# thetisproject/thetis

Hardware: AMD Instinct MI355X
Metric: DG element-updates/sec, 2D SWE DG-P1 SSPRK33 (higher is better)
Workload: dtype f64

## Files before the change

### thetis_amd/csrc/swe2d_api_fuse.hip

```cpp
#include "swe2d_handle.h"
#include "swe2d_fuse.h"

namespace swe2d_impl {

namespace {
typedef void (*fuse_kernel_t)(const SweFuseArgs);
template <bool SRC>
fuse_kernel_t pick_fuse_src(bool nl, bool lf)
{
    if (nl) return lf ? swe_fuse12_kernel<true, true, SRC> : swe_fuse12_kernel<true, false, SRC>;
    return lf ? swe_fuse12_kernel<false, true, SRC> : swe_fuse12_kernel<false, false, SRC>;
}
fuse_kernel_t pick_fuse_kernel(bool nl, bool lf, bool src) { return src ? pick_fuse_src<true>(nl, lf) : pick_fuse_src<false>(nl, lf); }
}

int fuseq_build(Handle *h);
int fuse12_build(Handle *h)
{
    if (h->npc == 4) return fuseq_build(h);
    if (h->fuse_tile || h->fuse_state == -1 || stream_capturing(h)) return SWE2D_OK;
    const int n = h->n_cells;
    const size_t S = h->stride;
    const int *nbr = h->h_nbr.data();
    std::vector<int2> tl;
// ... 128 lines not shown
        const int ni = (int)cells.size();
        for (int c : ring) if (state[c] == 2) cells.push_back(c);
        const int nt = (int)cells.size();
        if (nt - ni != n_ring || nt > SWE_FUSE_WG) return fail(h, SWE2D_ERR_UNSUPPORTED, "fused stage pair: tile bookkeeping");
        for (int l = 0; l < nt; l++) lane_of[cells[l]] = l;
        const size_t base = tl.size();
        tl.resize(base + SWE_FUSE_WG, int4{-1, 0, 0, 0});
        int n_out = 0;
        for (int l = 0; l < nt; l++) {
            const int c = cells[l];
            unsigned w[4];
            for (int f = 0; f < 4; f++) {
                const int code = nbr[(size_t)f*S + c];
                if (code < 0) w[f] = (unsigned)l;
                else if (state[code >> 2] != 0) w[f] = (unsigned)lane_of[code >> 2];
                else {
                    if (l < ni || n_out >= SWE_QFUSE_MAX_OUT) return fail(h, SWE2D_ERR_UNSUPPORTED, "fused stage pair: ring bookkeeping");
                    w[f] = 0x200u | (unsigned)n_out++;
                }
            }
            tl[base + l] = int4{c, (int)(w[0] | (w[1] << SWE_FUSE_FBITS) | (w[2] << (2*SWE_FUSE_FBITS))), (int)w[3], 0};
        }
        inner.push_back(ni);
        n_ring_total += nt - ni;
        for (int c : cells) { state[c] = 0; lane_of[c] = -1; }
    }
    h->fuseq_n_tiles = (int)inner.size();
    if (!fuse12_tiles_pay(h, h->fuseq_n_tiles)) { h->fuse_state = -1; h->fuseq_n_tiles = 0; return SWE2D_OK; }
    HIP_TRY(h, hipMalloc(&h->fuseq_tile, tl.size()*sizeof(int4)));
    HIP_TRY(h, hipMalloc(&h->fuseq_inner, inner.size()*sizeof(int)));
    HIP_TRY(h, hipMemcpy(h->fuseq_tile, tl.data(), tl.size()*sizeof(int4), hipMemcpyHostToDevice));
    HIP_TRY(h, hipMemcpy(h->fuseq_inner, inner.data(), inner.size()*sizeof(int), hipMemcpyHostToDevice));
    h->fuseq_ring_cells = n_ring_total;
    return SWE2D_OK;
}

namespace {
typedef void (*fuseq_kernel_t)(const SweFuseQuadArgs);
template <bool SRC, bool AFFINE>
fuseq_kernel_t pick_fuseq_2(bool nl, bool lf)
{
    if (nl) return lf ? swe_fuse12_quad_kernel<true, true, SRC, AFFINE> : swe_fuse12_quad_kernel<true, false, SRC, AFFINE>;
    return lf ? swe_fuse12_quad_kernel<false, true, SRC, AFFINE> : swe_fuse12_quad_kernel<false, false, SRC, AFFINE>;
}
fuseq_kernel_t pick_fuseq_kernel(bool nl, bool lf, bool src, bool affine)
{
    if (affine) return src ? pick_fuseq_2<true, true>(nl, lf) : pick_fuseq_2<false, true>(nl, lf);
    return src ? pick_fuseq_2<true, false>(nl, lf) : pick_fuseq_2<false, false>(nl, lf);
}
}

int launch_fuse12_quad(Handle *h, int cell_end)
{
    if (!h->fuseq_tile) return fail(h, SWE2D_ERR_UNSUPPORTED, "fused stage pair: no tile tables");
    SweFuseQuadArgs q;
    fill_stage_args(h, q.st, 0, 0, 2, 0.0, 1.0, kBeta[0], 0, h->n_owned);
    q.tile = h->fuseq_tile;
    q.n_inner = h->fuseq_inner;
    q.n_tiles = h->fuseq_n_tiles;
    q.cell_end = cell_end;
    q.beta1 = kBeta[0];
    q.a0_2 = kAlpha0[1]; q.a1_2 = kAlphaIn[1]; q.beta2 = kBeta[1];
    q.out = h->state[2];
    fuseq_kernel_t kern = pick_fuseq_kernel(h->par.use_nonlinear_equations != 0, h->par.use_lax_friedrichs_velocity != 0, has_sources(h), h->affine);
    const int grid = ((h->fuseq_n_tiles + 7)/8)*8;
    SWE_CHK_SYNC(h->stream);
    hipLaunchKernelGGL(kern, dim3(grid), dim3(SWE_FUSE_WG), 0, h->stream, q);
    HIP_TRY(h, hipGetLastError());
    stage_written(h, false, true);
    return SWE2D_OK;
}

namespace {
typedef void (*fuse3_kernel_t)(const SweFuse3Args);
template <bool SRC>
fuse3_kernel_t pick_fuse3_src(bool nl, bool lf)
{
    if (nl) return lf ? swe_fuse123_kernel<true, true, SRC> : swe_fuse123_kernel<true, false, SRC>;
    return lf ? swe_fuse123_kernel<false, true, SRC> : swe_fuse123_kernel<false, false, SRC>;
}
fuse3_kernel_t pick_fuse3_kernel(bool nl, bool lf, bool src) { return src ? pick_fuse3_src<true>(nl, lf) : pick_fuse3_src<false>(nl, lf); }
}

int fuse123_build(Handle *h)
{
    if (h->fuse3_tile || stream_capturing(h)) return SWE2D_OK;
    const int n = h->n_cells;
    const size_t S = h->stride;
    const int *nbr = h->h_nbr.data();
    const int *order = (int)h->fuse3_order.size() == n ? h->fuse3_order.data() : ((int)h->fuse_order.size() == n ? h->fuse_order.data() : nullptr);
    const unsigned char *start = (int)h->fuse3_start.size() == n ? h->fuse3_start.data() : nullptr;
    std::vector<int2> tl, cnt;
    std::vector<unsigned char> state((size_t)n, 0);
    std::vector<int> lane_of((size_t)n, -1), touched, inner;
    std::vector<std::pair<int, unsigned char>> undo;
    int count[4] = {0, 0, 0, 0};
    long long r1_total = 0, r2_total = 0;
    auto set = [&](int c, unsigned char ns) {
        undo.push_back({c, state[c]});
        if (state[c] == 0) touched.push_back(c);
        count[state[c]]--; state[c] = ns; count[ns]++;
    };
    for (int pos = 0; pos < n;) {
        inner.clear(); touched.clear();
        count[1] = count[2] = count[3] = 0;
        while (pos < n) {
            if (start && start[pos] && !inner.empty()) break;
            const int kk = order ? order[pos] : pos;
            undo.clear();
            const size_t touched_before = touched.size();
            set(kk, 1);
            for (int f = 0; f < 3; f++) {
                const int code = nbr[(size_t)f*S + kk];
                if (code < 0) continue;
                const int c1 = code >> 2;
                if (state[c1] == 0 || state[c1] == 3) {
                    set(c1, 2);
                    for (int g = 0; g < 3; g++) {
                        const int code2 = nbr[(size_t)g*S + c1];
                        if (code2 >= 0 && state[code2 >> 2] == 0) set(code2 >> 2, 3);
                    }
                }
            }
            if (count[1] + count[2] + count[3] > SWE_FUSE_WG || 2*count[3] > SWE_FUSE3_MAX_OUT) {
                if (inner.empty()) return fail(h, SWE2D_ERR_UNSUPPORTED, "fused stages: a cell whose two rings do not fit a tile");
                for (size_t i = undo.size(); i-- > 0;) { count[state[undo[i].first]]--; state[undo[i].first] = undo[i].second; count[undo[i].second]++; }
                touched.resize(touched_before);
                break;
            }
            inner.push_back(kk);
            pos++;
        }
        std::vector<int> cells(inner);
        for (int want = 2; want <= 3; want++)
            for (int c : touched) if (state[c] == want) cells.push_back(c);
        const int ni = (int)inner.size(), nm = ni + count[2], nt = (int)cells.size();
        if (nt != count[1] + count[2] + count[3] || ni != count[1] || nt > SWE_FUSE_WG) return fail(h, SWE2D_ERR_UNSUPPORTED, "fused stages: tile bookkeeping");
        for (int l = 0; l < nt; l++) lane_of[cells[l]] = l;
        const size_t base = tl.size();
        tl.resize(base + SWE_FUSE_WG, int2{-1, 0});
        int n_out = 0;
        for (int l = 0; l < nt; l++) {
            const int c = cells[l];
            unsigned w = 0u;
            for (int f = 0; f < 3; f++) {
                const int code = nbr[(size_t)f*S + c];
                unsigned field;
                if (code < 0) field = (unsigned)l;
                else if (state[code >> 2] != 0) field = (unsigned)lane_of[code >> 2];
                else {
                    if (l < nm || n_out >= SWE_FUSE3_MAX_OUT) return fail(h, SWE2D_ERR_UNSUPPORTED, "fused stages: ring bookkeeping");
                    field = 0x200u | (unsigned)n_out++;
                }
                w |= field << (SWE_FUSE_FBITS*f);
            }
            tl[base + l] = int2{c, (int)w};
        }
        cnt.push_back(int2{ni, nm});
        r1_total += count[2]; r2_total += count[3];
        for (int c : cells) { state[c] = 0; lane_of[c] = -1; }
    }
    h->fuse3_n_tiles = (int)cnt.size();
    HIP_TRY(h, hipMalloc(&h->fuse3_tile, tl.size()*sizeof(int2)));
    HIP_TRY(h, hipMalloc(&h->fuse3_cnt, cnt.size()*sizeof(int2)));
    HIP_TRY(h, hipMemcpy(h->fuse3_tile, tl.data(), tl.size()*sizeof(int2), hipMemcpyHostToDevice));
    HIP_TRY(h, hipMemcpy(h->fuse3_cnt, cnt.data(), cnt.size()*sizeof(int2), hipMemcpyHostToDevice));
    h->fuse3_ring1 = r1_total; h->fuse3_ring2 = r2_total;
    return SWE2D_OK;
}

int launch_fuse123(Handle *h, int cell_end)
{
    if (int rc = capture_parity_check(h)) return rc;
    if (int rc = fuse123_build(h)) return rc;
    if (!h->fuse3_tile) return fail(h, SWE2D_ERR_UNSUPPORTED, "fused stages: no tile tables (not built inside a stream capture)");
    SweFuse3Args q;
    fill_stage_args(h, q.st, 0, 0, 1, 0.0, 1.0, kBeta[0], 0, h->n_owned);
    q.st.idxc = h->opt[SWE2D_OPT_COMPACT_IDX] == 0 ? nullptr : h->idxc;
    q.tile = h->fuse3_tile;
    q.counts = h->fuse3_cnt;
    q.n_tiles = h->fuse3_n_tiles;
    q.cell_end = cell_end;
    for (int s = 0; s < 3; s++) { q.a0[s] = s ? kAlpha0[s] : 0.0; q.a1[s] = s ? kAlphaIn[s] : 1.0; q.beta[s] = kBeta[s]; }
    q.out = h->state[1];
    fuse3_kernel_t kern = pick_fuse3_kernel(h->par.use_nonlinear_equations != 0, h->par.use_lax_friedrichs_velocity != 0, has_sources(h));
    const int grid = ((h->fuse3_n_tiles + 7)/8)*8;
    SWE_CHK_SYNC(h->stream);
    hipLaunchKernelGGL(kern, dim3(grid), dim3(SWE_FUSE_WG), 0, h->stream, q);
    HIP_TRY(h, hipGetLastError());
    swap_state_buffers(h);
    unsigned long long id = 0;
    if (stream_capturing(h, &id)) {
        if (id != h->capture_id) { h->capture_id = id; h->capture_swaps = 0; }
        h->capture_swaps++;
    }
    return SWE2D_OK;
}

int capture_parity_check(Handle *h)
{
    if (h->capture_swaps == 0 && h->capture_odd == 0) return SWE2D_OK;
    unsigned long long id = 0;
    const bool capturing = stream_capturing(h, &id);
    if (h->capture_swaps) {
        if (capturing && id == h->capture_id) return SWE2D_OK;
        if (h->capture_swaps & 1) { swap_state_buffers(h); h->capture_odd++; }
        h->capture_swaps = 0;
    }
    if (capturing || h->capture_odd == 0) return SWE2D_OK;
    const int odd = h->capture_odd;
    h->capture_odd = 0;
    return fail(h, SWE2D_ERR_UNSUPPORTED, std::to_string(odd) + " stream capture(s) recorded an odd number of swe2d_solve_step_cells launches: "
                "such a graph ends on the other state buffer than it began on and cannot be replayed (the state is the one from before the "
                "capture); capture an even number per sequence");
}

}

static int checked_tile_order(Handle *h, const int32_t *cells, std::vector<int> &order)
{
    std::vector<char> seen((size_t)h->n_cells, 0);
    for (int i = 0; cells && i < h->n_cells; i++) {
        if (cells[i] < 0 || cells[i] >= h->n_cells || seen[cells[i]]) return fail(h, SWE2D_ERR_INVALID_ARGUMENT, "fused stages: the tile order is not a permutation of the cells");
        seen[cells[i]] = 1;
    }
    if (cells) order.assign(cells, cells + h->n_cells);
    return SWE2D_OK;
}

extern "C" {

int swe2d_fused_set_order(swe2d_handle *hh, const int32_t *cells_in_tile_order)
{
    Handle *h = H(hh);
    if (!h) return SWE2D_ERR_INVALID_ARGUMENT;
    HIP_TRY(h, hipSetDevice(h->device));
    std::vector<int> order;
    if (int rc = checked_tile_order(h, cells_in_tile_order, order)) return rc;
    HIP_TRY(h, hipStreamSynchronize(h->stream));
    if (h->fuse_tile) { (void)hipFree(h->fuse_tile); h->fuse_tile = nullptr; }
    if (h->fuse_inner) { (void)hipFree(h->fuse_inner); h->fuse_inner = nullptr; }
// ... 80 lines not shown
```

### thetis_amd/csrc/swe2d_flow.h

```cpp
#pragma once
#include "swe2d_kernels.h"
#include "swe2d_p2p.h"

#ifndef SWE_FLOW_OCCUPANCY
#define SWE_FLOW_OCCUPANCY __attribute__((amdgpu_waves_per_eu(2, 2)))
#endif
#define SWE_FLOW_MAX_STAGES 384
#define SWE_FLOW_MAX_CYCLES 64
#ifndef SWE_FLOW_FLAG_STRIDE
#define SWE_FLOW_FLAG_STRIDE 16
#endif
#define SWE_FLOW_SLOT_BYTES 128
#define SWE_FLOW_DIV6(t_) ((int)(((unsigned)(t_)*43691u) >> 18))
#ifndef SWE_FLOW_POLL_SLEEP
#define SWE_FLOW_POLL_SLEEP 2
#endif
#ifndef SWE_FLOW_NTR_SRC
#define SWE_FLOW_NTR_SRC 3
#endif
#ifndef SWE_FLOW_WALLFAST_SRC
#define SWE_FLOW_WALLFAST_SRC true
#endif
#ifndef SWE_FLOW_RX
#define SWE_FLOW_RX 3
// ... 72 lines not shown
    while (wall_clock64() - t0 < (unsigned long long)ticks) __builtin_amdgcn_s_sleep(16);
    if (aux_sys) __builtin_amdgcn_raw_buffer_store_b64(lo2, r, off, 0, 17); else __builtin_amdgcn_raw_buffer_store_b64(lo2, r, off, 0, 16);
}
#define SWE_FLOW_TORN(lb_, pc_, sys_) ((swe_flow_tear[0] == (lb_) || swe_flow_tear[0] == -2) && swe_flow_tear[1] > 0 \
                                       && ((pc_) % (swe_flow_tear[2] < 1 ? 1 : swe_flow_tear[2])) == 0 && (!(sys_) || swe_flow_tear[3]))
#endif
__device__ __forceinline__ void swe_flow_put(__amdgpu_buffer_rsrc_t r, unsigned off, double x, unsigned tag, bool torn = false)
{
    const swe_u32x2 xb = __builtin_bit_cast(swe_u32x2, x);
    const swe_u32x4 g = {xb.x, xb.y, tag, swe_flow_check_word(xb.x, xb.y, tag)};
#ifdef SWE_FLOW_TEAR
    if (torn) { swe_flow_put_torn(r, off, g, 0, swe_flow_tear[1]); return; }
#endif
    (void)torn;
    __builtin_amdgcn_raw_buffer_store_b128(g, r, off, 0, 16);
}
__device__ __forceinline__ swe_u32x4 swe_flow_get(__amdgpu_buffer_rsrc_t r, unsigned off)
{
    return __builtin_amdgcn_raw_buffer_load_b128(r, off, 0, 16);
}
__device__ __forceinline__ void swe_flow_put_sys(__amdgpu_buffer_rsrc_t r, unsigned off, double x, unsigned tag, bool torn = false)
{
    const swe_u32x2 xb = __builtin_bit_cast(swe_u32x2, x);
    const swe_u32x4 g = {xb.x, xb.y, tag, swe_flow_check_word(xb.x, xb.y, tag)};
#ifdef SWE_FLOW_TEAR
    if (torn) { swe_flow_put_torn(r, off, g, 1, swe_flow_tear[1]); return; }
#endif
    (void)torn;
    __builtin_amdgcn_raw_buffer_store_b128(g, r, off, 0, 17);
}
__device__ __forceinline__ swe_u32x4 swe_flow_get_sys(__amdgpu_buffer_rsrc_t r, unsigned off)
{
    return __builtin_amdgcn_raw_buffer_load_b128(r, off, 0, 17);
}
__device__ __forceinline__ double swe_flow_val(swe_u32x4 g)
{
    const swe_u32x2 xb = {g.x, g.y};
    return __builtin_bit_cast(double, xb);
}
__device__ __forceinline__ bool swe_flow_arrived(swe_u32x4 g, unsigned need)
{
#ifdef SWE_FLOW_NOCHECK
    return (int)(g.z - need) >= 0;
#else
    return (int)(g.z - need) >= 0 && g.w == swe_flow_check_word(g.x, g.y, g.z);
#endif
}

template <bool NONLIN, bool WD = false>
__device__ __forceinline__ void swe_flow_rhs_cell(const SweStageArgs &p, const double u[3], const double v[3], const double e[3],
                                                  const double h[3], const double nx[3], const double ny[3], double bu[3], double bv[3],
                                                  double be[3], const double *Dn = nullptr)
{
#pragma clang fp contract(off)
    const double g = p.g;
    double H[3], gxs[3], gys[3];
#pragma unroll
    for (int i = 0; i < 3; i++) {
        H[i] = WD ? Dn[i] : (NONLIN ? h[i] + e[i] : h[i]);
        gxs[i] = -0.5*nx[(i + 1) % 3];
        gys[i] = -0.5*ny[(i + 1) % 3];
    }
    const double ge3 = g*(e[0] + e[1] + e[2])*(1.0/3.0);
    const double SHu = swe_int2(H, u)*(1.0/12.0), SHv = swe_int2(H, v)*(1.0/12.0);
#pragma unroll
    for (int i = 0; i < 3; i++) {
        bu[i] = gxs[i]*ge3;
        bv[i] = gys[i]*ge3;
        be[i] = swe_dot2(gxs[i], SHu, gys[i], SHv);
    }
    if (NONLIN) {
        const double Suu = swe_int2(u, u)*(1.0/12.0), Suv = swe_int2(u, v)*(1.0/12.0), Svv = swe_int2(v, v)*(1.0/12.0);
        const double D12 = fma(gys[2], v[2], fma(gys[1], v[1], fma(gys[0], v[0],
                           fma(gxs[2], u[2], fma(gxs[1], u[1], gxs[0]*u[0])))))*(1.0/12.0);
        const double us = u[0] + u[1] + u[2], vs = v[0] + v[1] + v[2];
#pragma unroll
        for (int i = 0; i < 3; i++) {
            bu[i] = fma(gys[i], Suv, fma(gxs[i], Suu, fma(D12, us + u[i], bu[i])));
            bv[i] = fma(gys[i], Svv, fma(gxs[i], Suv, fma(D12, vs + v[i], bv[i])));
        }
    }
}

template <bool NONLIN, bool LF, bool SRC, int NTR, bool WD = false, int XG = SWE_FLOW_XG, int PLANE = SWE_BLOCK, int NLDS = SWE_FLOW_LDS_DOUBLES>
__device__ __forceinline__ void swe_flow_rhs_facets(const SweStageArgs &p, int k, const double u[3], const double v[3], const double e[3],
                                                    const double h[3], const double *lds, const unsigned tr[3][NTR], int bmarkers,
                                                    const double nx[3], const double ny[3], double twoA, double bu[3], double bv[3],
                                                    double be[3], const double *Dn = nullptr, const double *al = nullptr)
{
#pragma clang fp contract(off)
    const double g = p.g;
#pragma unroll
    for (int f = 0; f < 3; f++) {
        const int a = f, b = (f + 1) % 3;
        const bool bnd = ((bmarkers >> (8*f)) & 0xff) != 0;
        const unsigned ab0 = tr[f][0] & 0xffffu, aa0 = tr[f][0] >> 16;
        const unsigned step = ab0 >= (unsigned)XG ? 1u : (unsigned)(3*PLANE);
        const unsigned ab1 = NTR == 3 ? tr[f][NTR - 2] & 0xffffu : ab0 + step, aa1 = NTR == 3 ? tr[f][NTR - 2] >> 16 : aa0 + step;
        const unsigned ab2 = NTR == 3 ? tr[f][NTR - 1] & 0xffffu : ab0 + 2u*step, aa2 = NTR == 3 ? tr[f][NTR - 1] >> 16 : aa0 + 2u*step;
        const double unb = lds[SWE_LDSI(ab0, NLDS)], una = lds[SWE_LDSI(aa0, NLDS)];
        const double vnb = lds[SWE_LDSI(ab1, NLDS)], vna = lds[SWE_LDSI(aa1, NLDS)];
        const double enb = lds[SWE_LDSI(ab2, NLDS)], ena = lds[SWE_LDSI(aa2, NLDS)];
        const double nxs = nx[f], nys = ny[f];
        double Lf, rLf;
        swe_sqrt_rsqrt(swe_dot2(nxs, nxs, nys, nys), Lf, rLf);
        double Fau, Fbu, Fav, Fbv, Fae, Fbe;
        if constexpr (WD) {
            const double ena_ = swe_wd_eta(ena, h[a], al[a]), enb_ = swe_wd_eta(enb, h[b], al[b]);
            swe_facet_flux<NONLIN, LF, true>(g, p.sigma_lf, u[a], u[b], v[a], v[b], e[a], e[b], h[a], h[b], Dn[a], Dn[b], una, unb, vna, vnb,
                                             ena_, enb_, ena, enb, nxs, nys, Lf, rLf, Fau, Fbu, Fav, Fbv, Fae, Fbe);
        } else
        swe_facet_flux<NONLIN, LF, false>(g, p.sigma_lf, u[a], u[b], v[a], v[b], e[a], e[b], h[a], h[b], 0.0, 0.0, una, unb, vna, vnb, ena, enb,
                                          0.0, 0.0, nxs, nys, Lf, rLf, Fau, Fbu, Fav, Fbv, Fae, Fbe);
        if (bnd) { Fau = 0.0; Fbu = 0.0; Fav = 0.0; Fbv = 0.0; Fae = 0.0; Fbe = 0.0; }
        bu[a] = fma(-0.5, Fau, bu[a]); bu[b] = fma(-0.5, Fbu, bu[b]);
        bv[a] = fma(-0.5, Fav, bv[a]); bv[b] = fma(-0.5, Fbv, bv[b]);
        be[a] = fma(-0.5, Fae, be[a]); be[b] = fma(-0.5, Fbe, be[b]);
    }
    if (SRC) {
        double H[3], gxs[3], gys[3];
#pragma unroll
        for (int i = 0; i < 3; i++) {
            H[i] = WD ? Dn[i] : (NONLIN ? h[i] + e[i] : h[i]);
            gxs[i] = -0.5*nx[(i + 1) % 3];
            gys[i] = -0.5*ny[(i + 1) % 3];
        }
        swe_source_terms(p, k, p.stride, twoA, u, v, H, gxs, gys, bu, bv, be);
    }
}

template <bool NONLIN, bool LF, bool WALLFAST, bool WD = false>
__device__ __forceinline__ void swe_flow_finish(const SweStageArgs &p, int k, double beta, const double u[3], const double v[3],
                                                const double e[3], const double h[3], const double nx[3], const double ny[3],
                                                double twoA, int bmarkers, int bkind1, const double bu[3], const double bv[3], const double be[3],
                                                const double wu[3], const double wv[3], const double we[3], double ou[3],
                                                double ov[3], double oe[3], const double *Dn = nullptr, const double *al = nullptr)
{
#pragma clang fp contract(off)
    const double s = 6.0*p.dt*beta*swe_rcp(twoA);
    const double su = bu[0] + bu[1] + bu[2], sv = bv[0] + bv[1] + bv[2], se = be[0] + be[1] + be[2];
#pragma unroll
    for (int i = 0; i < 3; i++) {
        ou[i] = fma(s, fma(4.0, bu[i], -su), wu[i]);
        ov[i] = fma(s, fma(4.0, bv[i], -sv), wv[i]);
        oe[i] = fma(s, fma(4.0, be[i], -se), we[i]);
    }
    if (bmarkers != 0) {
        const double sfac = 6.0*p.dt*beta*swe_rcp(fma(-ny[0], -nx[2], -(nx[0]*ny[2])));
        int rem = ((bmarkers & 0xff) ? 1 : 0) | ((bmarkers & 0xff00) ? 2 : 0) | ((bmarkers & 0xff0000) ? 4 : 0);
        int kind_next = bkind1;
        const double u_0 = u[0], u_1 = u[1], u_2 = u[2], v_0 = v[0], v_1 = v[1], v_2 = v[2], e_0 = e[0], e_1 = e[1], e_2 = e[2];
        const double h_0 = h[0], h_1 = h[1], h_2 = h[2], nx_0 = nx[0], nx_1 = nx[1], nx_2 = nx[2], ny_0 = ny[0], ny_1 = ny[1], ny_2 = ny[2];
        const double D_0 = WD ? Dn[0] : 0.0, D_1 = WD ? Dn[1] : 0.0, D_2 = WD ? Dn[2] : 0.0;
        const double al_0 = WD ? al[0] : 0.0, al_1 = WD ? al[1] : 0.0, al_2 = WD ? al[2] : 0.0;
#define SWE_SEL3(x, i) ((i) == 0 ? x##_0 : ((i) == 1 ? x##_1 : x##_2))
#pragma unroll 1
        while (rem) {
            const int f = (rem & 1) ? 0 : ((rem & 2) ? 1 : 2);
            rem &= rem - 1;
            const int a = f, b = (f == 2) ? 0 : f + 1;
            const double nxs = SWE_SEL3(nx, f), nys = SWE_SEL3(ny, f);
            double Lf, rLf;
            swe_sqrt_rsqrt(swe_dot2(nxs, nxs, nys, nys), Lf, rLf);
            double Fau = 0.0, Fbu = 0.0, Fav = 0.0, Fbv = 0.0, Fae = 0.0, Fbe = 0.0;
            const double Ha_ = WD ? SWE_SEL3(D, a) : (!NONLIN ? SWE_SEL3(h, a) : SWE_SEL3(h, a) + SWE_SEL3(e, a));
            const double Hb_ = WD ? SWE_SEL3(D, b) : (!NONLIN ? SWE_SEL3(h, b) : SWE_SEL3(h, b) + SWE_SEL3(e, b));
            swe_boundary_facet<NONLIN, LF, WD, WALLFAST>(p, (bmarkers >> (8*f)) & 0xff, k, a, b, SWE_SEL3(u, a), SWE_SEL3(u, b), SWE_SEL3(v, a),
                                                  SWE_SEL3(v, b), SWE_SEL3(e, a), SWE_SEL3(e, b), SWE_SEL3(h, a), SWE_SEL3(h, b),
                                                  Ha_, Hb_, WD ? SWE_SEL3(al, a) : 0.0, WD ? SWE_SEL3(al, b) : 0.0, nxs, nys, Lf, rLf, Fau, Fbu, Fav,
                                                  Fbv, Fae, Fbe, kind_next);
            kind_next = -1;
            const double dau = -0.5*Fau, dbu = -0.5*Fbu, dav = -0.5*Fav, dbv = -0.5*Fbv, dae = -0.5*Fae, dbe = -0.5*Fbe;
#pragma unroll
            for (int i = 0; i < 3; i++) {
                const double wa = (i == a) ? 3.0 : -1.0, wb = (i == b) ? 3.0 : -1.0;
                ou[i] = fma(sfac, fma(wa, dau, wb*dbu), ou[i]);
                ov[i] = fma(sfac, fma(wa, dav, wb*dbv), ov[i]);
                oe[i] = fma(sfac, fma(wa, dae, wb*dbe), oe[i]);
            }
        }
#undef SWE_SEL3
    }
    if constexpr (WD) swe_wd_finish<3>(p.g, beta*p.dt, h, al, ou, ov, oe, !p.wd_skip_relax);
}

#ifdef SWE_WAVE_TIMING
#ifndef SWE_FLOW_TS_STAGE
#define SWE_FLOW_TS_STAGE 7
#endif
#define SWE_FT(i) do { if (s == SWE_FLOW_TS_STAGE && lane == 0 && lb < SWE_WT_MAX) swe_wave_ts[i][lb] = wall_clock64(); } while (0)
#else
#define SWE_FT(i)
#endif


template <bool NONLIN, bool LF, bool SRC, bool FX, int POLL = 6, bool WD = false>
__global__ __launch_bounds__(SWE_BLOCK) SWE_FLOW_OCCUPANCY void swe_flow_kernel(const SweFlowArgs q)
{
#pragma clang fp contract(off)
    __shared__ double lds[SWE_FLOW_LDS_DOUBLES];
    __shared__ int xsrc[SWE_FLOW_MAX_RIM];
    __shared__ int lact[SWE_BLOCK];
    __shared__ unsigned lrec[SWE_BLOCK];
    __shared__ int lpeer[SWE_BLOCK];
    __shared__ unsigned char lpub[SWE_FLOW_MAX_RIM];
    __shared__ double lu0[9][SWE_BLOCK];
    const SweStageArgs &p = q.st;
    const int lb = swe_logical_block(blockIdx.x, gridDim.x);
    if (lb >= q.n_blocks) return;
    const int lane = (int)threadIdx.x;
    const int kcode = q.fcell[lb*SWE_BLOCK + lane];
    const bool real = kcode >= 0;
    const int k = real ? kcode : -1 - kcode;
    const size_t S = p.stride;
    const unsigned S8 = (unsigned)S*8u;
    unsigned *const myflag = q.flag + (size_t)lb*SWE_FLOW_FLAG_STRIDE;
    const unsigned base = *myflag;
    const unsigned fin = base + (unsigned)q.n_stages;
    if (!FX && !__any(real && k < q.cell_end[0])) {
        if (lane == 0) *myflag = fin;
        return;
    }
// ... 462 lines not shown
```

### thetis_amd/csrc/swe2d_fuse.h

```cpp
#pragma once
#include "swe2d_kernels.h"
#include "swe2d_flow.h"

#ifndef SWE_FUSE_WG
#define SWE_FUSE_WG 256
#endif
#ifndef SWE_FUSE_MIN_WG
#define SWE_FUSE_MIN_WG 3
#endif
#ifndef SWE_FUSE_INNER
#define SWE_FUSE_INNER 192
#endif
#define SWE_FUSE_FBITS 10
#define SWE_FUSE_RING (SWE_FUSE_WG - SWE_FUSE_INNER)
#define SWE_FUSE_XG (9*SWE_FUSE_WG)
#define SWE_FUSE_MAX_OUT (2*SWE_FUSE_RING)
#define SWE_FUSE_LDS (SWE_FUSE_XG + 6*SWE_FUSE_MAX_OUT)

struct SweFuseArgs {
    SweStageArgs st;
    const int2 *tile;
    const int *n_inner;
    int n_tiles;
    int cell_end;
// ... 54 lines not shown
            const int code = outside[f] ? nbf : ((k << 2) | f);
            const unsigned kn8 = (unsigned)(code >> 2)*8u;
            const int g2 = code & 3;
            const unsigned ob = kn8 + (g2 == 0 ? 0u : (g2 == 1 ? S8 : 2u*S8));
            const unsigned oa = kn8 + (g2 == 0 ? S8 : (g2 == 1 ? 2u*S8 : 0u));
            r0[f][0] = swe_ld(gu, ob, 0); r0[f][1] = swe_ld(gv, ob, 0); r0[f][2] = swe_ld(ge, ob, 0);
            r0[f][3] = swe_ld(gu, oa, 0); r0[f][4] = swe_ld(gv, oa, 0); r0[f][5] = swe_ld(ge, oa, 0);
        }
        double px[3], py[3];
        const swe_rsrc_t rvx = swe_rsrc(p.vx), rvy = swe_rsrc(p.vy), rvh = swe_rsrc(p.vh);
#pragma unroll
        for (int i = 0; i < 3; i++) {
            const unsigned v8 = (unsigned)vid[i]*8u;
            px[i] = swe_ld(rvx, v8, 0);
            py[i] = swe_ld(rvy, v8, 0);
            h[i] = swe_ld(rvh, v8, 0);
        }
#pragma unroll
        for (int f = 0; f < 3; f++) {
            const int b = (f + 1) % 3;
            nx[f] = py[b] - py[f];
            ny[f] = px[f] - px[b];
        }
#pragma unroll
        for (int i = 0; i < 3; i++) { lds[i*SWE_FUSE_WG + lane] = u[i]; lds[(3 + i)*SWE_FUSE_WG + lane] = v[i]; lds[(6 + i)*SWE_FUSE_WG + lane] = e[i]; }
#pragma unroll
        for (int f = 0; f < 3; f++) {
            if (outside[f]) {
                const unsigned at = ((unsigned)tl.y >> (SWE_FUSE_FBITS*f)) & 0x1ffu;
#pragma unroll
                for (int j = 0; j < 6; j++) lds[SWE_LDSI(SWE_FUSE_XG + 6*at + j, SWE_FUSE_LDS)] = r0[f][j];
            }
        }
    }
    __syncthreads();
    double o1u[3], o1v[3], o1e[3];
    double twoA = 0.0;
    if (real) {
        twoA = fma(nx[0], ny[1], -(ny[0]*nx[1]));
        double bu[3], bv[3], be[3], wu[3], wv[3], we[3];
        swe_flow_rhs_cell<NONLIN>(p, u, v, e, h, nx, ny, bu, bv, be);
        swe_flow_rhs_facets<NONLIN, LF, SRC, 1, false, SWE_FUSE_XG, SWE_FUSE_WG, SWE_FUSE_LDS>(p, k, u, v, e, h, lds, tr, bmarkers, nx, ny, twoA, bu, bv, be);
#pragma unroll
        for (int i = 0; i < 3; i++) { wu[i] = 1.0*u[i]; wv[i] = 1.0*v[i]; we[i] = 1.0*e[i]; }
        swe_flow_finish<NONLIN, LF, true>(p, k, q.beta1, u, v, e, h, nx, ny, twoA, bmarkers, bkind1, bu, bv, be, wu, wv, we, o1u, o1v, o1e);
    }
    __syncthreads();
    if (real) {
#pragma unroll
        for (int i = 0; i < 3; i++) { lds[i*SWE_FUSE_WG + lane] = o1u[i]; lds[(3 + i)*SWE_FUSE_WG + lane] = o1v[i]; lds[(6 + i)*SWE_FUSE_WG + lane] = o1e[i]; }
    }
    const bool act2 = lane < n_inner && k < q.cell_end;
    if (act2) {
#pragma unroll
        for (int i = 0; i < 3; i++) {
            lw[i][lane] = fma(q.a0_2, u[i], q.a1_2*o1u[i]);
            lw[3 + i][lane] = fma(q.a0_2, v[i], q.a1_2*o1v[i]);
            lw[6 + i][lane] = fma(q.a0_2, e[i], q.a1_2*o1e[i]);
        }
    }
    __syncthreads();
    if (act2) {
#pragma unroll
        for (int i = 0; i < 3; i++) asm volatile("" : "+v"(nx[i]), "+v"(ny[i]), "+v"(h[i]));
#pragma unroll
        for (int f = 0; f < 3; f++) asm volatile("" : "+v"(tr[f][0]));
        asm volatile("" : "+v"(bmarkers), "+v"(twoA));
        double bu[3], bv[3], be[3], wu[3], wv[3], we[3], ou[3], ov[3], oe[3];
        swe_flow_rhs_cell<NONLIN>(p, o1u, o1v, o1e, h, nx, ny, bu, bv, be);
        swe_flow_rhs_facets<NONLIN, LF, SRC, 1, false, SWE_FUSE_XG, SWE_FUSE_WG, SWE_FUSE_LDS>(p, k, o1u, o1v, o1e, h, lds, tr, bmarkers, nx, ny, twoA, bu, bv, be);
#pragma unroll
        for (int i = 0; i < 3; i++) { wu[i] = lw[i][lane]; wv[i] = lw[3 + i][lane]; we[i] = lw[6 + i][lane]; }
        swe_flow_finish<NONLIN, LF, true>(p, k, q.beta2, o1u, o1v, o1e, h, nx, ny, twoA, bmarkers, bkind1, bu, bv, be, wu, wv, we, ou, ov, oe);
        const swe_rsrc_t gou = swe_rsrc(q.out), gov = swe_rsrc(q.out + 3*S), goe = swe_rsrc(q.out + 6*S);
#pragma unroll
        for (int i = 0; i < 3; i++) {
            swe_st(gou, k8, i*S8, ou[i]);
            swe_st(gov, k8, i*S8, ov[i]);
            swe_st(goe, k8, i*S8, oe[i]);
        }
    }
}

#define SWE_FUSE3_XG (18*SWE_FUSE_WG)
#ifndef SWE_FUSE3_MAX_OUT
#define SWE_FUSE3_MAX_OUT 224
#endif
#define SWE_FUSE3_LDS (SWE_FUSE3_XG + 6*SWE_FUSE3_MAX_OUT)
#ifndef SWE_FUSE3_SRC_MIN_WG
#define SWE_FUSE3_SRC_MIN_WG 2
#endif

struct SweFuse3Args {
    SweStageArgs st;
    const int2 *tile;
    const int2 *counts;
    int n_tiles;
    int cell_end;
    double a0[3], a1[3], beta[3];
    double *out;
};

template <bool NONLIN, bool LF, bool SRC = false>
__global__ __launch_bounds__(SWE_FUSE_WG, SRC ? SWE_FUSE3_SRC_MIN_WG : SWE_FUSE_MIN_WG) void swe_fuse123_kernel(const SweFuse3Args q)
{
#pragma clang fp contract(off)
    __shared__ double lds[SWE_FUSE3_LDS];
    const SweStageArgs &p = q.st;
    const int tile = swe_logical_block(blockIdx.x, gridDim.x);
    if (tile >= q.n_tiles) return;
    const int lane = (int)threadIdx.x;
    const int2 tl = q.tile[(size_t)tile*SWE_FUSE_WG + lane];
    const bool real = tl.x >= 0;
    const int k = real ? tl.x : 0;
    const int2 cnt = q.counts[tile];
    const size_t S = p.stride;
    const unsigned S8 = (unsigned)S*8u, k8 = (unsigned)k*8u;
    double *const P1 = lds + 9*SWE_FUSE_WG;

    int bmarkers = 0, bkind1 = 0;
    unsigned tr[3][1];
    double h[3], nx[3], ny[3], u[3], v[3], e[3];
    if (real) {
        int nb[3], vid[3];
        swe_conn_load(p.idxc, p.idx4, p.idx2, k, nb, vid);
        bmarkers = (nb[0] < 0 ? -nb[0] : 0) | (nb[1] < 0 ? (-nb[1]) << 8 : 0) | (nb[2] < 0 ? (-nb[2]) << 16 : 0);
        if (bmarkers != 0) {
            const int m1 = (bmarkers & 0xff) ? (bmarkers & 0xff) : ((bmarkers & 0xff00) ? ((bmarkers >> 8) & 0xff) : (bmarkers >> 16));
            bkind1 = m1 < SWE_MAX_MARKERS ? p.bc.kind[m1] : 0;
        }
        const swe_rsrc_t gu = swe_rsrc(p.uin), gv = swe_rsrc(p.uin + 3*S), ge = swe_rsrc(p.uin + 6*S);
#pragma unroll
        for (int i = 0; i < 3; i++) {
            u[i] = swe_ld(gu, k8, i*S8);
            v[i] = swe_ld(gv, k8, i*S8);
            e[i] = swe_ld(ge, k8, i*S8);
        }
        double r0[3][6];
        bool outside[3];
#pragma unroll
        for (int f = 0; f < 3; f++) {
            const int nbf = nb[f];
            const unsigned w = ((unsigned)tl.y >> (SWE_FUSE_FBITS*f)) & 0x3ffu;
            outside[f] = (w & 0x200u) != 0u;
            const unsigned at = w & 0x1ffu;
            const int f2 = nbf >= 0 ? (nbf & 3) : f, f2a = f2 == 2 ? 0 : f2 + 1;
            {
                const unsigned ab = outside[f] ? (unsigned)(SWE_FUSE3_XG + 6*at) : (unsigned)(f2*SWE_FUSE_WG + at);
                const unsigned aa = outside[f] ? (unsigned)(SWE_FUSE3_XG + 6*at + 3) : (unsigned)(f2a*SWE_FUSE_WG + at);
                tr[f][0] = ab | (aa << 16);
            }
            const int code = outside[f] ? nbf : ((k << 2) | f);
            const unsigned kn8 = (unsigned)(code >> 2)*8u;
            const int g2 = code & 3;
            const unsigned ob = kn8 + (g2 == 0 ? 0u : (g2 == 1 ? S8 : 2u*S8));
            const unsigned oa = kn8 + (g2 == 0 ? S8 : (g2 == 1 ? 2u*S8 : 0u));
            r0[f][0] = swe_ld(gu, ob, 0); r0[f][1] = swe_ld(gv, ob, 0); r0[f][2] = swe_ld(ge, ob, 0);
            r0[f][3] = swe_ld(gu, oa, 0); r0[f][4] = swe_ld(gv, oa, 0); r0[f][5] = swe_ld(ge, oa, 0);
        }
        double px[3], py[3];
        const swe_rsrc_t rvx = swe_rsrc(p.vx), rvy = swe_rsrc(p.vy), rvh = swe_rsrc(p.vh);
#pragma unroll
        for (int i = 0; i < 3; i++) {
            const unsigned v8 = (unsigned)vid[i]*8u;
            px[i] = swe_ld(rvx, v8, 0);
            py[i] = swe_ld(rvy, v8, 0);
            h[i] = swe_ld(rvh, v8, 0);
        }
#pragma unroll
        for (int f = 0; f < 3; f++) {
            const int b = (f + 1) % 3;
            nx[f] = py[b] - py[f];
            ny[f] = px[f] - px[b];
        }
#pragma unroll
        for (int i = 0; i < 3; i++) { lds[i*SWE_FUSE_WG + lane] = u[i]; lds[(3 + i)*SWE_FUSE_WG + lane] = v[i]; lds[(6 + i)*SWE_FUSE_WG + lane] = e[i]; }
#pragma unroll
        for (int f = 0; f < 3; f++) {
            if (outside[f]) {
                const unsigned at = ((unsigned)tl.y >> (SWE_FUSE_FBITS*f)) & 0x1ffu;
#pragma unroll
                for (int j = 0; j < 6; j++) lds[SWE_LDSI(SWE_FUSE3_XG + 6*at + j, SWE_FUSE3_LDS)] = r0[f][j];
            }
        }
    }
    __syncthreads();
    double twoA = 0.0;
    if (real) {
        twoA = fma(nx[0], ny[1], -(ny[0]*nx[1]));
        double bu[3], bv[3], be[3], wu[3], wv[3], we[3], ou[3], ov[3], oe[3];
        swe_flow_rhs_cell<NONLIN>(p, u, v, e, h, nx, ny, bu, bv, be);
        swe_flow_rhs_facets<NONLIN, LF, SRC, 1, false, SWE_FUSE3_XG, SWE_FUSE_WG, SWE_FUSE3_LDS>(p, k, u, v, e, h, lds, tr, bmarkers, nx, ny, twoA, bu, bv, be);
#pragma unroll
        for (int i = 0; i < 3; i++) { wu[i] = 1.0*u[i]; wv[i] = 1.0*v[i]; we[i] = 1.0*e[i]; }
        swe_flow_finish<NONLIN, LF, true>(p, k, q.beta[0], u, v, e, h, nx, ny, twoA, bmarkers, bkind1, bu, bv, be, wu, wv, we, ou, ov, oe);
#pragma unroll
        for (int i = 0; i < 3; i++) { u[i] = ou[i]; v[i] = ov[i]; e[i] = oe[i]; }
#pragma unroll
        for (int i = 0; i < 3; i++) { P1[i*SWE_FUSE_WG + lane] = u[i]; P1[(3 + i)*SWE_FUSE_WG + lane] = v[i]; P1[(6 + i)*SWE_FUSE_WG + lane] = e[i]; }
    }
    __syncthreads();
#pragma unroll 1
    for (int s = 1; s < 3; s++) {
        const bool act = lane < (s == 1 ? cnt.y : cnt.x) && (s == 1 || k < q.cell_end);
        double ou[3], ov[3], oe[3];
        if (act) {
#pragma unroll
            for (int i = 0; i < 3; i++) asm volatile("" : "+v"(nx[i]), "+v"(ny[i]), "+v"(h[i]));
#pragma unroll
            for (int f = 0; f < 3; f++) asm volatile("" : "+v"(tr[f][0]));
            asm volatile("" : "+v"(bmarkers), "+v"(twoA));
            double bu[3], bv[3], be[3], wu[3], wv[3], we[3];
            swe_flow_rhs_cell<NONLIN>(p, u, v, e, h, nx, ny, bu, bv, be);
            swe_flow_rhs_facets<NONLIN, LF, SRC, 1, false, SWE_FUSE3_XG, SWE_FUSE_WG, 9*SWE_FUSE_WG>(p, k, u, v, e, h, P1, tr, bmarkers, nx, ny, twoA, bu, bv, be);
            const double a0 = q.a0[s], a1 = q.a1[s];
#pragma unroll
            for (int i = 0; i < 3; i++) {
                wu[i] = fma(a0, lds[i*SWE_FUSE_WG + lane], a1*u[i]);
                wv[i] = fma(a0, lds[(3 + i)*SWE_FUSE_WG + lane], a1*v[i]);
                we[i] = fma(a0, lds[(6 + i)*SWE_FUSE_WG + lane], a1*e[i]);
            }
            swe_flow_finish<NONLIN, LF, true>(p, k, q.beta[s], u, v, e, h, nx, ny, twoA, bmarkers, bkind1, bu, bv, be, wu, wv, we, ou, ov, oe);
        }
        if (s == 1) {
            __syncthreads();
            if (act) {
#pragma unroll
                for (int i = 0; i < 3; i++) { P1[i*SWE_FUSE_WG + lane] = ou[i]; P1[(3 + i)*SWE_FUSE_WG + lane] = ov[i]; P1[(6 + i)*SWE_FUSE_WG + lane] = oe[i]; }
#pragma unroll
                for (int i = 0; i < 3; i++) { u[i] = ou[i]; v[i] = ov[i]; e[i] = oe[i]; }
            }
            __syncthreads();
        } else if (act) {
            const swe_rsrc_t gou = swe_rsrc(q.out), gov = swe_rsrc(q.out + 3*S), goe = swe_rsrc(q.out + 6*S);
#pragma unroll
            for (int i = 0; i < 3; i++) {
                swe_st(gou, k8, i*S8, ou[i]);
                swe_st(gov, k8, i*S8, ov[i]);
                swe_st(goe, k8, i*S8, oe[i]);
            }
        }
    }
}


#define SWE_QFUSE_INNER 192
#define SWE_QFUSE_RING (SWE_FUSE_WG - SWE_QFUSE_INNER)
#define SWE_QFUSE_XG (12*SWE_FUSE_WG)
#define SWE_QFUSE_MAX_OUT (3*SWE_QFUSE_RING)
#define SWE_QFUSE_LDS (SWE_QFUSE_XG + 6*SWE_QFUSE_MAX_OUT)

struct SweFuseQuadArgs {
    SweStageArgs st;
    const int4 *tile;
    const int *n_inner;
    int n_tiles;
    int cell_end;
    double beta1, a0_2, a1_2, beta2;
    double *out;
};

template <bool NONLIN, bool LF, bool SRC, bool AFFINE>
__global__ __launch_bounds__(SWE_FUSE_WG, SWE_FUSE_MIN_WG) void swe_fuse12_quad_kernel(const SweFuseQuadArgs q)
{
#pragma clang fp contract(off)
    __shared__ double lds[SWE_QFUSE_LDS];
    __shared__ double lu0[12*SWE_QFUSE_INNER];
    const SweStageArgs &p = q.st;
    const int tile = swe_logical_block(blockIdx.x, gridDim.x);
    if (tile >= q.n_tiles) return;
    const int lane = (int)threadIdx.x;
    const int4 tl = q.tile[(size_t)tile*SWE_FUSE_WG + lane];
    const bool real = tl.x >= 0;
    const int k = real ? tl.x : 0;
    const int n_inner = q.n_inner[tile];
    const size_t S = p.stride;
    const unsigned S8 = (unsigned)S*8u, k8 = (unsigned)k*8u, S4 = (unsigned)S*4u, k4 = (unsigned)k*4u;

    unsigned tr[4] = {0u, 0u, 0u, 0u}, bmarkers = 0u;
    int nb[4] = {-1, -1, -1, -1}, vid[4] = {0, 0, 0, 0};
    double u[4], v[4], e[4];
    if (real) {
#pragma unroll
        for (int i = 0; i < 4; i++) {
            nb[i] = swe_ldi(swe_rsrc(p.nbr), k4, i*S4);
            vid[i] = swe_ldi(swe_rsrc(p.cv), k4, i*S4);
        }
        const swe_rsrc_t gu = swe_rsrc(p.uin), gv = swe_rsrc(p.uin + 4*S), ge = swe_rsrc(p.uin + 8*S);
#pragma unroll
        for (int i = 0; i < 4; i++) {
            u[i] = swe_ld(gu, k8, i*S8);
            v[i] = swe_ld(gv, k8, i*S8);
            e[i] = swe_ld(ge, k8, i*S8);
        }
        bmarkers = (nb[0] < 0 ? (unsigned)(-nb[0]) : 0u) | (nb[1] < 0 ? (unsigned)(-nb[1]) << 8 : 0u) |
                   (nb[2] < 0 ? (unsigned)(-nb[2]) << 16 : 0u) | (nb[3] < 0 ? (unsigned)(-nb[3]) << 24 : 0u);
        double r0[4][6];
        bool outside[4];
#pragma unroll
        for (int f = 0; f < 4; f++) {
            const int nbf = nb[f];
            const unsigned w = f < 3 ? (((unsigned)tl.y >> (SWE_FUSE_FBITS*f)) & 0x3ffu) : ((unsigned)tl.z & 0x3ffu);
            outside[f] = (w & 0x200u) != 0u;
            const unsigned at = w & 0x1ffu;
            const int f2 = nbf >= 0 ? (nbf & 3) : f, na = (f2 + 1) & 3;
            const unsigned ab = outside[f] ? (unsigned)(SWE_QFUSE_XG + 6*at) : (unsigned)(f2*SWE_FUSE_WG + at);
            const unsigned aa = outside[f] ? (unsigned)(SWE_QFUSE_XG + 6*at + 3) : (unsigned)(na*SWE_FUSE_WG + at);
            tr[f] = ab | (aa << 16);
            const int code = outside[f] ? nbf : ((k << 2) | f);
            const unsigned kn8 = (unsigned)(code >> 2)*8u;
            const int g2 = code & 3, ga = (g2 + 1) & 3;
            const unsigned ob = kn8 + ((g2 & 1) ? S8 : 0u) + ((g2 & 2) ? 2u*S8 : 0u);
            const unsigned oa = kn8 + ((ga & 1) ? S8 : 0u) + ((ga & 2) ? 2u*S8 : 0u);
            r0[f][0] = swe_ld(gu, ob, 0); r0[f][1] = swe_ld(gv, ob, 0); r0[f][2] = swe_ld(ge, ob, 0);
            r0[f][3] = swe_ld(gu, oa, 0); r0[f][4] = swe_ld(gv, oa, 0); r0[f][5] = swe_ld(ge, oa, 0);
        }
#pragma unroll
        for (int i = 0; i < 4; i++) { lds[i*SWE_FUSE_WG + lane] = u[i]; lds[(4 + i)*SWE_FUSE_WG + lane] = v[i]; lds[(8 + i)*SWE_FUSE_WG + lane] = e[i]; }
#pragma unroll
        for (int f = 0; f < 4; f++) {
            if (outside[f]) {
                const unsigned at = (f < 3 ? ((unsigned)tl.y >> (SWE_FUSE_FBITS*f)) : (unsigned)tl.z) & 0x1ffu;
#pragma unroll
                for (int j = 0; j < 6; j++) lds[SWE_LDSI(SWE_QFUSE_XG + 6*at + j, SWE_QFUSE_LDS)] = r0[f][j];
            }
// ... 48 lines not shown
```

Before: 30.89 billion.

## Cache per-cell facet geometry in LDS and rotate tile lanes across waves

In the three-stage fused SSPRK kernel, the first stage now stores each cell's facet lengths, their reciprocals and the reciprocal area in LDS, and stages two and three read them back instead of recomputing sqrt and reciprocal. To make room, the exchange area is shrunk to reuse the P1 region, and twoA no longer has to stay live in a register. The tile builder also rotates the lane assignment per tile by a hashed multiple of 64, so the active inner and ring cells land on different wavefronts from tile to tile. This is meant to spread the partial-activity stages 2 and 3 across waves. It adds an extra barrier and optional wave-timing instrumentation.

```diff
diff --git a/thetis_amd/csrc/swe2d_api_fuse.hip b/thetis_amd/csrc/swe2d_api_fuse.hip
--- a/thetis_amd/csrc/swe2d_api_fuse.hip
+++ b/thetis_amd/csrc/swe2d_api_fuse.hip
@@ -234,6 +234,9 @@
 fuse3_kernel_t pick_fuse3_kernel(bool nl, bool lf, bool src) { return src ? pick_fuse3_src<true>(nl, lf) : pick_fuse3_src<false>(nl, lf); }
 }
 
+#ifndef SWE_FUSE3_ROT
+#define SWE_FUSE3_ROT(tile) ((int)(((unsigned)(tile)*0x9E3779B1u) >> 30))
+#endif
 int fuse123_build(Handle *h)
 {
     if (h->fuse3_tile || stream_capturing(h)) return SWE2D_OK;
@@ -288,7 +291,9 @@
             for (int c : touched) if (state[c] == want) cells.push_back(c);
         const int ni = (int)inner.size(), nm = ni + count[2], nt = (int)cells.size();
         if (nt != count[1] + count[2] + count[3] || ni != count[1] || nt > SWE_FUSE_WG) return fail(h, SWE2D_ERR_UNSUPPORTED, "fused stages: tile bookkeeping");
-        for (int l = 0; l < nt; l++) lane_of[cells[l]] = l;
+        const int rot = SWE_FUSE3_ROT((int)cnt.size()) & 3;
+        auto phys = [rot](int role) { return (role + 64*rot) & (SWE_FUSE_WG - 1); };
+        for (int l = 0; l < nt; l++) lane_of[cells[l]] = phys(l);
         const size_t base = tl.size();
         tl.resize(base + SWE_FUSE_WG, int2{-1, 0});
         int n_out = 0;
@@ -298,7 +303,7 @@
             for (int f = 0; f < 3; f++) {
                 const int code = nbr[(size_t)f*S + c];
                 unsigned field;
-                if (code < 0) field = (unsigned)l;
+                if (code < 0) field = (unsigned)phys(l);
                 else if (state[code >> 2] != 0) field = (unsigned)lane_of[code >> 2];
                 else {
                     if (l < nm || n_out >= SWE_FUSE3_MAX_OUT) return fail(h, SWE2D_ERR_UNSUPPORTED, "fused stages: ring bookkeeping");
@@ -306,9 +311,9 @@
                 }
                 w |= field << (SWE_FUSE_FBITS*f);
             }
-            tl[base + l] = int2{c, (int)w};
-        }
-        cnt.push_back(int2{ni, nm});
+            tl[base + phys(l)] = int2{c, (int)w};
+        }
+        cnt.push_back(int2{ni, nm | (rot << 16)});
         r1_total += count[2]; r2_total += count[3];
         for (int c : cells) { state[c] = 0; lane_of[c] = -1; }
     }
diff --git a/thetis_amd/csrc/swe2d_flow.h b/thetis_amd/csrc/swe2d_flow.h
--- a/thetis_amd/csrc/swe2d_flow.h
+++ b/thetis_amd/csrc/swe2d_flow.h
@@ -178,11 +178,15 @@
     }
 }
 
-template <bool NONLIN, bool LF, bool SRC, int NTR, bool WD = false, int XG = SWE_FLOW_XG, int PLANE = SWE_BLOCK, int NLDS = SWE_FLOW_LDS_DOUBLES>
+#define SWE_GEOM_COMPUTE 0
+#define SWE_GEOM_KEEP 1
+#define SWE_GEOM_STORED 2
+template <bool NONLIN, bool LF, bool SRC, int NTR, bool WD = false, int XG = SWE_FLOW_XG, int PLANE = SWE_BLOCK, int NLDS = SWE_FLOW_LDS_DOUBLES,
+          int GEOM = SWE_GEOM_COMPUTE>
 __device__ __forceinline__ void swe_flow_rhs_facets(const SweStageArgs &p, int k, const double u[3], const double v[3], const double e[3],
                                                     const double h[3], const double *lds, const unsigned tr[3][NTR], int bmarkers,
                                                     const double nx[3], const double ny[3], double twoA, double bu[3], double bv[3],
-                                                    double be[3], const double *Dn = nullptr, const double *al = nullptr)
+                                                    double be[3], const double *Dn = nullptr, const double *al = nullptr, double *geo = nullptr)
 {
 #pragma clang fp contract(off)
     const double g = p.g;
@@ -199,7 +203,9 @@
         const double enb = lds[SWE_LDSI(ab2, NLDS)], ena = lds[SWE_LDSI(aa2, NLDS)];
         const double nxs = nx[f], nys = ny[f];
         double Lf, rLf;
-        swe_sqrt_rsqrt(swe_dot2(nxs, nxs, nys, nys), Lf, rLf);
+        if constexpr (GEOM == SWE_GEOM_STORED) { Lf = geo[f*PLANE]; rLf = geo[(3 + f)*PLANE]; }
+        else swe_sqrt_rsqrt(swe_dot2(nxs, nxs, nys, nys), Lf, rLf);
+        if constexpr (GEOM == SWE_GEOM_KEEP) { geo[f*PLANE] = Lf; geo[(3 + f)*PLANE] = rLf; }
         double Fau, Fbu, Fav, Fbv, Fae, Fbe;
         if constexpr (WD) {
             const double ena_ = swe_wd_eta(ena, h[a], al[a]), enb_ = swe_wd_eta(enb, h[b], al[b]);
@@ -225,15 +231,21 @@
     }
 }
 
-template <bool NONLIN, bool LF, bool WALLFAST, bool WD = false>
+template <bool NONLIN, bool LF, bool WALLFAST, bool WD = false, int GEOM = SWE_GEOM_COMPUTE, int PLANE = SWE_BLOCK>
 __device__ __forceinline__ void swe_flow_finish(const SweStageArgs &p, int k, double beta, const double u[3], const double v[3],
                                                 const double e[3], const double h[3], const double nx[3], const double ny[3],
                                                 double twoA, int bmarkers, int bkind1, const double bu[3], const double bv[3], const double be[3],
                                                 const double wu[3], const double wv[3], const double we[3], double ou[3],
-                                                double ov[3], double oe[3], const double *Dn = nullptr, const double *al = nullptr)
+                                                double ov[3], double oe[3], const double *Dn = nullptr, const double *al = nullptr,
+                                                double *geo = nullptr)
 {
 #pragma clang fp contract(off)
-    const double s = 6.0*p.dt*beta*swe_rcp(twoA);
+    const double dtb6 = 6.0*p.dt*beta;
+    double rA;
+    if constexpr (GEOM == SWE_GEOM_STORED) rA = geo[6*PLANE];
+    else rA = swe_rcp(twoA);
+    if constexpr (GEOM == SWE_GEOM_KEEP) geo[6*PLANE] = rA;
+    const double s = dtb6*rA;
     const double su = bu[0] + bu[1] + bu[2], sv = bv[0] + bv[1] + bv[2], se = be[0] + be[1] + be[2];
 #pragma unroll
     for (int i = 0; i < 3; i++) {
diff --git a/thetis_amd/csrc/swe2d_fuse.h b/thetis_amd/csrc/swe2d_fuse.h
--- a/thetis_amd/csrc/swe2d_fuse.h
+++ b/thetis_amd/csrc/swe2d_fuse.h
@@ -160,11 +160,17 @@
     }
 }
 
-#define SWE_FUSE3_XG (18*SWE_FUSE_WG)
 #ifndef SWE_FUSE3_MAX_OUT
 #define SWE_FUSE3_MAX_OUT 224
 #endif
-#define SWE_FUSE3_LDS (SWE_FUSE3_XG + 6*SWE_FUSE3_MAX_OUT)
+#ifndef SWE_FUSE3_GEOM
+#define SWE_FUSE3_GEOM 1
+#endif
+#define SWE_FUSE3_NGEO 7
+#define SWE_FUSE3_GEO (18*SWE_FUSE_WG)
+#define SWE_FUSE3_XG (SWE_FUSE3_GEOM ? 9*SWE_FUSE_WG : 18*SWE_FUSE_WG)
+#define SWE_FUSE3_LDS (SWE_FUSE3_GEOM ? SWE_FUSE3_GEO + SWE_FUSE3_NGEO*SWE_FUSE_WG : SWE_FUSE3_XG + 6*SWE_FUSE3_MAX_OUT)
+static_assert(6*SWE_FUSE3_MAX_OUT <= 9*SWE_FUSE_WG, "the staging area must fit P1");
 #ifndef SWE_FUSE3_SRC_MIN_WG
 #define SWE_FUSE3_SRC_MIN_WG 2
 #endif
@@ -192,9 +198,13 @@
     const bool real = tl.x >= 0;
     const int k = real ? tl.x : 0;
     const int2 cnt = q.counts[tile];
+    const int n_inner = cnt.x, n_mid = cnt.y & 0xffff, rot64 = (cnt.y >> 16) << 6;
     const size_t S = p.stride;
     const unsigned S8 = (unsigned)S*8u, k8 = (unsigned)k*8u;
     double *const P1 = lds + 9*SWE_FUSE_WG;
+#ifdef SWE_WAVE_TIMING
+    int wt_bodies = __any(real) ? 1 : 0;
+#endif
 
     int bmarkers = 0, bkind1 = 0;
     unsigned tr[3][1];
@@ -263,34 +273,47 @@
         }
     }
     __syncthreads();
+    constexpr int GEOM1 = SWE_FUSE3_GEOM ? SWE_GEOM_KEEP : SWE_GEOM_COMPUTE, GEOM23 = SWE_FUSE3_GEOM ? SWE_GEOM_STORED : SWE_GEOM_COMPUTE;
     double twoA = 0.0;
+    double *const G = lds + SWE_FUSE3_GEO + lane;
     if (real) {
         twoA = fma(nx[0], ny[1], -(ny[0]*nx[1]));
         double bu[3], bv[3], be[3], wu[3], wv[3], we[3], ou[3], ov[3], oe[3];
         swe_flow_rhs_cell<NONLIN>(p, u, v, e, h, nx, ny, bu, bv, be);
-        swe_flow_rhs_facets<NONLIN, LF, SRC, 1, false, SWE_FUSE3_XG, SWE_FUSE_WG, SWE_FUSE3_LDS>(p, k, u, v, e, h, lds, tr, bmarkers, nx, ny, twoA, bu, bv, be);
+        swe_flow_rhs_facets<NONLIN, LF, SRC, 1, false, SWE_FUSE3_XG, SWE_FUSE_WG, SWE_FUSE3_LDS, GEOM1>(p, k, u, v, e, h, lds, tr, bmarkers, nx, ny, twoA, bu, bv, be,
+                                                                                                     nullptr, nullptr, G);
 #pragma unroll
         for (int i = 0; i < 3; i++) { wu[i] = 1.0*u[i]; wv[i] = 1.0*v[i]; we[i] = 1.0*e[i]; }
-        swe_flow_finish<NONLIN, LF, true>(p, k, q.beta[0], u, v, e, h, nx, ny, twoA, bmarkers, bkind1, bu, bv, be, wu, wv, we, ou, ov, oe);
+        swe_flow_finish<NONLIN, LF, true, false, GEOM1, SWE_FUSE_WG>(p, k, q.beta[0], u, v, e, h, nx, ny, twoA, bmarkers, bkind1, bu, bv, be, wu, wv, we, ou, ov, oe,
+                                                        nullptr, nullptr, G);
 #pragma unroll
         for (int i = 0; i < 3; i++) { u[i] = ou[i]; v[i] = ov[i]; e[i] = oe[i]; }
+    }
+    if (SWE_FUSE3_GEOM) __syncthreads();
+    if (real) {
 #pragma unroll
         for (int i = 0; i < 3; i++) { P1[i*SWE_FUSE_WG + lane] = u[i]; P1[(3 + i)*SWE_FUSE_WG + lane] = v[i]; P1[(6 + i)*SWE_FUSE_WG + lane] = e[i]; }
     }
     __syncthreads();
 #pragma unroll 1
     for (int s = 1; s < 3; s++) {
-        const bool act = lane < (s == 1 ? cnt.y : cnt.x) && (s == 1 || k < q.cell_end);
+        const int role = (lane - rot64) & (SWE_FUSE_WG - 1);
+        const bool act = role < (s == 1 ? n_mid : n_inner) && (s == 1 || k < q.cell_end);
+#ifdef SWE_WAVE_TIMING
+        wt_bodies += __any(act) ? 1 : 0;
+#endif
         double ou[3], ov[3], oe[3];
         if (act) {
 #pragma unroll
             for (int i = 0; i < 3; i++) asm volatile("" : "+v"(nx[i]), "+v"(ny[i]), "+v"(h[i]));
 #pragma unroll
             for (int f = 0; f < 3; f++) asm volatile("" : "+v"(tr[f][0]));
-            asm volatile("" : "+v"(bmarkers), "+v"(twoA));
+            asm volatile("" : "+v"(bmarkers));
+            if (SRC || !SWE_FUSE3_GEOM) asm volatile("" : "+v"(twoA));
             double bu[3], bv[3], be[3], wu[3], wv[3], we[3];
             swe_flow_rhs_cell<NONLIN>(p, u, v, e, h, nx, ny, bu, bv, be);
-            swe_flow_rhs_facets<NONLIN, LF, SRC, 1, false, SWE_FUSE3_XG, SWE_FUSE_WG, 9*SWE_FUSE_WG>(p, k, u, v, e, h, P1, tr, bmarkers, nx, ny, twoA, bu, bv, be);
+            swe_flow_rhs_facets<NONLIN, LF, SRC, 1, false, SWE_FUSE3_XG, SWE_FUSE_WG, 9*SWE_FUSE_WG, GEOM23>(p, k, u, v, e, h, P1, tr, bmarkers, nx, ny, twoA, bu, bv, be,
+                                                                                                          nullptr, nullptr, G);
             const double a0 = q.a0[s], a1 = q.a1[s];
 #pragma unroll
             for (int i = 0; i < 3; i++) {
@@ -298,7 +321,8 @@
                 wv[i] = fma(a0, lds[(3 + i)*SWE_FUSE_WG + lane], a1*v[i]);
                 we[i] = fma(a0, lds[(6 + i)*SWE_FUSE_WG + lane], a1*e[i]);
             }
-            swe_flow_finish<NONLIN, LF, true>(p, k, q.beta[s], u, v, e, h, nx, ny, twoA, bmarkers, bkind1, bu, bv, be, wu, wv, we, ou, ov, oe);
+            swe_flow_finish<NONLIN, LF, true, false, GEOM23, SWE_FUSE_WG>(p, k, q.beta[s], u, v, e, h, nx, ny, twoA, bmarkers, bkind1, bu, bv, be, wu, wv, we, ou, ov, oe,
+                                                                          nullptr, nullptr, G);
         }
         if (s == 1) {
             __syncthreads();
@@ -319,6 +343,15 @@
             }
         }
     }
+#ifdef SWE_WAVE_TIMING
+    if ((lane & 63) == 0 && 4*blockIdx.x + (lane >> 6) < 6*SWE_WT_MAX) {
+        unsigned hw, xcc;
+        asm volatile("s_getreg_b32 %0, hwreg(HW_REG_HW_ID)" : "=s"(hw));
+        asm volatile("s_getreg_b32 %0, hwreg(HW_REG_XCC_ID)" : "=s"(xcc));
+        (&swe_wave_ts[0][0])[4*blockIdx.x + (lane >> 6)] = (unsigned long long)hw | ((unsigned long long)(xcc & 0xf) << 32)
+                                                           | ((unsigned long long)wt_bodies << 40) | (1ull << 44);
+    }
+#endif
 }
 
 
```

Result: faster. 32.02 billion (median of 6 runs) (+3.7%).
